# egor-achkasov/hermespy-rt

Hardware: AMD Instinct MI355X
Metric: resolved propagation paths/sec (higher is better)
Workload: dtype f32; 1 GPU; simple_street_canyon_with_cars.hrt, 1 TX + 4 RX, 4000000 rays/TX, 4 bounces, 3.5 GHz; parallelism=ray-sharded x1 (weak scaling), round-robin 4096-path granules, rays_total=4000000

## Files before the change

hermespy-rt_amd/csrc/hrt_kernels.hip:

```cpp
#include <hip/hip_runtime.h>
#include <string.h>

#include <stdint.h>
#include <stdio.h>
#include <stdlib.h>

#include "hrt_kparams.h"
#include "hrt_launch_dir.h"
#include "hrt_libm.h"

#pragma clang fp contract(off)

namespace {

constexpr float kEps = 1.1920928955078125e-07f;
constexpr float kOnePlusEps = 1.00000011920928955078125f;
constexpr float kPi = 3.14159265358979323846f;
constexpr float kC = 299792458.0f;
constexpr float kInvC = 1.0f / kC;
__device__ __forceinline__ float div_c(float a)
{
    const float q = a * kInvC;
    const float r = __builtin_fmaf(-q, kC, a);
    return __builtin_fmaf(r, kInvC, q);
// ... 434 lines not shown
                const float nt_s = xor_sign(nt, sg);                                            \
                rm |= HRT_BALLOT(nt_s < kK5 * a) | HRT_BALLOT(nt_s > (best * a) * kK2);         \
                if (rm != ~0ull) {                                                              \
                    HRT_STAT(kind, 5, 1);                                                       \
                    const float u = nu / det;                                                   \
                    const float v = nv / det;                                                   \
                    const float w = u + v;                                                      \
                    const float dist = nt / det;                                                \
                    const bool rej = (rm >> lane) & 1ull;                                       \
                    const bool miss = (det > -kEps && det < kEps) | (u < -kEps) |               \
                                      (u > kOnePlusEps) | (v < -kEps) | (w > kOnePlusEps);      \
                    const uint32_t oj = orig[(J)];         \
                    const bool take = !rej & !miss & (dist > kEps) &                            \
                                      ((dist < best) | ((dist == best) & (oj < who_o)));        \
                    best = take ? dist : best;                                                  \
                    who = take ? (J) : who;                                                     \
                    who_o = take ? oj : who_o;                                                  \
                }                                                                               \
            }                                                                                   \
        }                                                                                       \
    }

constexpr uint32_t kMaskRounds = 16;
constexpr uint32_t kCandBuf = 64u;
__host__ __device__ constexpr uint32_t wave_scratch4(bool cand_buf) { return 2u * kMaskRounds + (cand_buf ? 4u * kCandBuf : 0u); }

__device__ __forceinline__ uint32_t rxt_cell(F3 a)
{
    const float ax = fabsf(a.x), ay = fabsf(a.y), az = fabsf(a.z);
    uint32_t m = 0u;
    float major = a.x, c1 = a.y, c2 = a.z;
    if (ay > ax && ay >= az) { m = 1u; major = a.y; c1 = a.z; c2 = a.x; }
    else if (az > ax && az > ay) { m = 2u; major = a.z; c1 = a.x; c2 = a.y; }
    const float inv = __builtin_amdgcn_rcpf(major);
    const float u = c1 * inv, v = c2 * inv;
    int iu = (int)((u * 0.5f + 0.5f) * (float)HRT_RXT_N), iv = (int)((v * 0.5f + 0.5f) * (float)HRT_RXT_N);
    iu = iu < 0 ? 0 : (iu > HRT_RXT_N - 1 ? HRT_RXT_N - 1 : iu);
    iv = iv < 0 ? 0 : (iv > HRT_RXT_N - 1 ? HRT_RXT_N - 1 : iv);
    const uint32_t f = m + (major < 0.f ? 3u : 0u);
    return (f * HRT_RXT_N + (uint32_t)iv) * HRT_RXT_N + (uint32_t)iu;
}

__device__ __forceinline__ bool rxt_inside(const hrt_krxt &X, F3 o)
{
    const F3 dc = sub3(o, {X.cx, X.cy, X.cz});
    return fast_sqrt(fdot3(dc, dc)) * 1.0001f <= X.region_r;
}
__device__ __forceinline__ unsigned long long rxt_cell_load(const hrt_krxt &X, uint32_t apex_k, F3 d)
{
    return X.cell_mask[(uint64_t)apex_k * HRT_RXT_BINS + rxt_cell(d)];
}
template <typename TriPtr>
__device__ __forceinline__ Hit closest_hit_masked(TriPtr tri, const uint32_t *__restrict__ orig, const hrt_krxt &X,
                                                  uint32_t apex_k, uint32_t num_tri, F3 o, F3 d, bool valid,
                                                  uint32_t lane, [[maybe_unused]] int kind)
{
    float best = 1e9f;
    uint32_t who = HRT_NO_HIT, who_o = 0u;
    const unsigned long long inval = HRT_BALLOT(!valid);
    if (inval == ~0ull) return {who, best};
    unsigned long long mine = 0ull;
    if (valid) {
        mine = rxt_inside(X, o) ? rxt_cell_load(X, apex_k, d)
                                : (num_tri >= 64u ? ~0ull : ((1ull << num_tri) - 1ull));
    }
    unsigned long long m = wave_or64(mine);
    HRT_STAT(kind, 0, 1);
    HRT_STAT(kind, 1, 1);
    HRT_STAT(kind, 2, __popcll(m));
    while (m) {
        const uint32_t j = (uint32_t)__builtin_ctzll(m);
        m &= m - 1ull;
        HRT_STAGED_BODY(j)
    }
    return {who, best};
}

using Rsrc = __amdgpu_buffer_rsrc_t;
__device__ __forceinline__ Rsrc make_rsrc(const uint8_t *base)
{
    return __builtin_amdgcn_make_buffer_rsrc(const_cast<uint8_t *>(base), 0, 0xffffffff, 0x00020000);
}

__device__ __forceinline__ void wave_or256(uint32_t (&w)[8])
{
    uint32_t c[4];
#pragma unroll
    for (int k = 0; k < 4; ++k) {
        const auto r = __builtin_amdgcn_permlane32_swap(w[k], w[k + 4], false, false);
        c[k] = (uint32_t)r[0] | (uint32_t)r[1];
    }
    uint32_t e[2];
#pragma unroll
    for (int k = 0; k < 2; ++k) {
        const auto r = __builtin_amdgcn_permlane16_swap(c[k], c[k + 2], false, false);
        e[k] = (uint32_t)r[0] | (uint32_t)r[1];
    }
#define HRT_OR2(CTRL) "v_or_b32_dpp %0, %0, %0 " CTRL "\n" "v_or_b32_dpp %1, %1, %1 " CTRL "\n" "s_nop 0\n"
    asm volatile(
        "s_nop 4\n"
        HRT_OR2("row_shr:1 row_mask:0xf bank_mask:0xf")
        HRT_OR2("row_shr:2 row_mask:0xf bank_mask:0xf")
        HRT_OR2("row_shr:4 row_mask:0xf bank_mask:0xf")
        HRT_OR2("row_shr:8 row_mask:0xf bank_mask:0xf")
        "s_nop 1\n"
        : "+v"(e[0]), "+v"(e[1]));
#undef HRT_OR2
#pragma unroll
    for (int k = 0; k < 8; ++k) w[k] = (uint32_t)__builtin_amdgcn_readlane((int)e[k & 1], 15 + 16 * (k >> 1));
}

__device__ __forceinline__ F3 image_of(F3 t, float4 q0, float4 q2)
{
    const F3 n = {q2.y, q2.z, q2.w};
    const float dn = fdot3(sub3(t, {q0.x, q0.y, q0.z}), n);
    return {__builtin_fmaf(-2.f * dn, n.x, t.x), __builtin_fmaf(-2.f * dn, n.y, t.y), __builtin_fmaf(-2.f * dn, n.z, t.z)};
}

struct PatchRef { bool served; uint32_t off; };
__device__ __forceinline__ void patch_fetch(const hrt_kpatch &X, uint32_t num_tri, uint32_t htri, bool valid, float4 &p0, float4 &p1)
{
    p0 = make_float4(0.f, 0.f, 0.f, 0.f);
    p1 = p0;
    if (valid && htri < num_tri) {
        p0 = reinterpret_cast<const float4 *>(X.pdef)[2u * htri];
        p1 = reinterpret_cast<const float4 *>(X.pdef)[2u * htri + 1u];
    }
}
template <typename TriPtr>
__device__ __forceinline__ PatchRef patch_locate(TriPtr tri, const hrt_kpatch &X, uint32_t num_tri, uint32_t htri, F3 o,
                                                 const bool image, F3 apex, F3 d, const float4 p0, const float4 p1)
{
    PatchRef R = {false, 0u};
    if (htri < num_tri) {
        const float4 q0 = tri[HRT_ROW * htri], q2 = tri[HRT_ROW * htri + 2];
        const F3 sv = sub3(o, {q0.x, q0.y, q0.z});
        const float fu = fdot3(sv, {p0.x, p0.y, p0.z}), fv = fdot3(sv, {p1.x, p1.y, p1.z});
        const float hh = fdot3(sv, {q2.y, q2.z, q2.w});
        const uint32_t bits = __float_as_uint(p1.w), nu = bits & 0xffffu, nv = bits >> 16;
        R.served = (nu != 0u) & (fabsf(hh) <= X.hmax) & (fu >= -HRT_PATCH_ACCEPT) & (fv >= -HRT_PATCH_ACCEPT) &
                   (fu <= (float)nu + HRT_PATCH_ACCEPT) & (fv <= (float)nv + HRT_PATCH_ACCEPT);
        if (image) {
            const F3 im = image_of(apex, q0, q2);
            const F3 wv = sub3(o, im);
            const F3 cx = fcross3(wv, d);
            R.served &= (fdot3(cx, cx) <= 0.98f * X.ro_img * X.ro_img) && (fdot3(wv, d) > 0.f);
        }
        const uint32_t iu = min((uint32_t)max((int)floorf(fu), 0), nu - 1u);
        const uint32_t iv = min((uint32_t)max((int)floorf(fv), 0), nv - 1u);
        R.off = (__float_as_uint(p0.w) + iv * nu + iu) * (HRT_PATCH_WORDS * 8u);
    }
    return R;
}

__device__ __forceinline__ void patch_load(const hrt_kpatch &X, const PatchRef R, uint32_t apex_k, bool valid, uint32_t (&w)[8])
{
#pragma unroll
    for (int k = 0; k < 8; ++k) w[k] = 0u;
    if (valid && R.served) {
        const Rsrc mr = make_rsrc(reinterpret_cast<const uint8_t *>(X.mask));
        const uint32_t off = R.off + apex_k * X.num_patch * (HRT_PATCH_WORDS * 8u);
        const auto a = __builtin_amdgcn_raw_buffer_load_b128(mr, (int)off, 0, 0);
        const auto b = __builtin_amdgcn_raw_buffer_load_b128(mr, (int)(off + 16u), 0, 0);
        w[0] = (uint32_t)a[0]; w[1] = (uint32_t)a[1]; w[2] = (uint32_t)a[2]; w[3] = (uint32_t)a[3];
        w[4] = (uint32_t)b[0]; w[5] = (uint32_t)b[1]; w[6] = (uint32_t)b[2]; w[7] = (uint32_t)b[3];
    }
}
__device__ __forceinline__ bool patch_whole(const PatchRef R, bool valid) { return HRT_BALLOT(valid && !R.served) != 0ull; }

template <typename TriPtr, typename OrigPtr>
__device__ __forceinline__ Hit closest_hit_words(TriPtr tri, OrigPtr orig, uint32_t (&w)[8], const bool whole, uint32_t num_tri,
                                                 F3 o, F3 d, bool valid, uint32_t lane, [[maybe_unused]] int kind)
{
    float best = 1e9f;
    uint32_t who = HRT_NO_HIT, who_o = 0u;
    const unsigned long long inval = HRT_BALLOT(!valid);
    if (inval == ~0ull) return {who, best};
    wave_or256(w);
    if (whole) {
#pragma unroll
        for (int k = 0; k < 8; ++k)
            w[k] |= num_tri >= 32u * (uint32_t)(k + 1) ? ~0u : (num_tri > 32u * (uint32_t)k ? (1u << (num_tri - 32u * (uint32_t)k)) - 1u : 0u);
    }
    HRT_STAT(kind, 0, 1);
    HRT_STAT(kind, 1, 1);
#pragma unroll
    for (uint32_t r = 0; r < HRT_PATCH_WORDS; ++r) {
        unsigned long long m = ((unsigned long long)w[2u * r + 1u] << 32) | (unsigned long long)w[2u * r];
        HRT_STAT(kind, 2, __popcll(m));
        while (m) {
            const uint32_t j = r * 64u + (uint32_t)__builtin_ctzll(m);
            m &= m - 1ull;
            HRT_STAGED_BODY(j)
        }
    }
    return {who, best};
}

template <typename TriPtr, typename OrigPtr>
__device__ __forceinline__ Hit closest_hit_patch(TriPtr tri, OrigPtr orig, const hrt_kpatch &X,
                                                 const PatchRef R, uint32_t apex_k, uint32_t num_tri, F3 o, F3 d,
                                                 bool valid, uint32_t lane, [[maybe_unused]] int kind)
{
    uint32_t w[8];
    patch_load(X, R, apex_k, valid, w);
    HRT_STAT(kind, 6, (valid && R.served) ? 1 : 0);
    return closest_hit_words(tri, orig, w, patch_whole(R, valid), num_tri, o, d, valid, lane, kind);
}

__device__ __forceinline__ void txcell_load(const hrt_kpatch &X, uint32_t tx, F3 d, uint32_t (&w)[8])
{
    const Rsrc mr = make_rsrc(reinterpret_cast<const uint8_t *>(X.txcell));
    const uint32_t off = (tx * HRT_RXT_BINS + rxt_cell(d)) * (HRT_PATCH_WORDS * 8u);
    const auto a = __builtin_amdgcn_raw_buffer_load_b128(mr, (int)off, 0, 0);
    const auto b = __builtin_amdgcn_raw_buffer_load_b128(mr, (int)(off + 16u), 0, 0);
    w[0] = (uint32_t)a[0]; w[1] = (uint32_t)a[1]; w[2] = (uint32_t)a[2]; w[3] = (uint32_t)a[3];
    w[4] = (uint32_t)b[0]; w[5] = (uint32_t)b[1]; w[6] = (uint32_t)b[2]; w[7] = (uint32_t)b[3];
}

template <typename TriPtr, typename OrigPtr>
__device__ __forceinline__ Hit closest_hit_txcell(TriPtr tri, OrigPtr orig, const hrt_kpatch &X, uint32_t tx, uint32_t num_tri,
                                                  F3 o, F3 d, bool valid, uint32_t lane)
{
    uint32_t w[8];
#pragma unroll
    for (int k = 0; k < 8; ++k) w[k] = 0u;
    if (valid) txcell_load(X, tx, d, w);
    return closest_hit_words(tri, orig, w, false, num_tri, o, d, valid, lane, 0);
}

template <bool MULTI, typename TriPtr>
__device__ __forceinline__ Hit closest_hit_packet(TriPtr tri, const uint32_t *__restrict__ orig,
                                                  const hrt_krxt &X, uint32_t rxk,
                                                  uint32_t num_tri, F3 o, F3 d,
                                                  bool valid, uint32_t lane, const Ball &B,
                                                  const bool shadow, F3 apex,
                                                  unsigned long long *wmask, int kind)
{
    float best = 1e9f;
    uint32_t who = HRT_NO_HIT, who_o = 0u;
    const unsigned long long inval = HRT_BALLOT(!valid);
    if (inval == ~0ull) return {who, best};
    uint32_t n_items = num_tri;
    const uint16_t *list = nullptr;
    Packet P0 = packet_bounds(B, d, valid, shadow, apex);
    HRT_STAT(kind, 0, 1);
    HRT_STAT(kind, 1, P0.usable ? 1 : 0);
    if ((shadow || (kind == 0 && X.num_txt != 0u)) && X.enabled && P0.usable) {
        const F3 dc = sub3(B.c, {X.cx, X.cy, X.cz});
        const bool inside = fast_sqrt(fdot3(dc, dc)) * 1.0001f + B.r <= X.region_r;
        float ro_apex = P0.ro;
        if (!shadow) ro_apex += (fabsf(B.c.x - apex.x) + fabsf(B.c.y - apex.y)) + fabsf(B.c.z - apex.z);
        if (inside && P0.sina <= HRT_RXT_SIN_AQ && ro_apex <= X.ro_bin[rxk]) {
            const uint32_t cell = (uint32_t)__builtin_amdgcn_readfirstlane((int)rxt_cell(P0.ax));
            const uint32_t e0 = X.off[rxk * HRT_RXT_BINS + cell], e1 = X.off[rxk * HRT_RXT_BINS + cell + 1u];
            list = X.idx + e0;
            n_items = e1 - e0;
            HRT_STAT(kind, 6, 1);
            HRT_STAT(kind, 7, n_items);
        }
    }
// ... 1568 lines not shown
                stf(hit_out(P, b), H_OZ * cap4, k4, o.z);
                stf(hit_out(P, b), H_DX * cap4, k4, d.x);
                stf(hit_out(P, b), H_DY * cap4, k4, d.y);
                stf(hit_out(P, b), H_DZ * cap4, k4, d.z);
                stf(hit_out(P, b), H_A0 * cap4, k4, a0);
                stf(hit_out(P, b), H_A1 * cap4, k4, a1);
                stf(hit_out(P, b), H_A2 * cap4, k4, a2);
                stf(hit_out(P, b), H_A3 * cap4, k4, a3);
                stf(hit_out(P, b), H_TAU * cap4, k4, tau);
            }
        }
    }
}

__global__ __launch_bounds__(HRT_BLOCK, 8) void hrt_image_kernel(const hrt_kparams P, const uint32_t b)
{
    extern __shared__ float4 lds[];
    const uint32_t tid = threadIdx.x, lane = tid & 63u;
    const uint32_t *counts = reinterpret_cast<const uint32_t *>(P.ws + P.off_counts);
    if (counts[P.num_bounces + 1] & kErrVoid) return;
    const uint32_t n_in = counts[b];
    const uint32_t n_chunks = (n_in + HRT_BLOCK - 1) / HRT_BLOCK;
    if (blockIdx.x >= n_chunks) return;
    const uint32_t T = P.num_tri;
    const uint32_t cap4 = (uint32_t)P.cap * 4u;
    float4 *l_tri = lds;
    uint32_t *l_wcnt = reinterpret_cast<uint32_t *>(lds + HRT_ROW * T);
    const uint32_t pb = b - 1;
    F3 o, d;
    uint32_t htri, hray;
    float4 pd0, pd1;
    const auto load_state = [&](const uint32_t chunk) {
        const uint32_t i = chunk * HRT_BLOCK + tid;
        const uint32_t i4 = i * 4u;
        o = {0.f, 0.f, 0.f};
        d = {0.f, 0.f, 1.f};
        htri = 0u;
        hray = 0u;
        if (i < n_in) {
            htri = ldu(hit_blk(P, pb), H_TRI * cap4, i4);
            o = {ldf(hit_blk(P, pb), H_OX * cap4, i4), ldf(hit_blk(P, pb), H_OY * cap4, i4), ldf(hit_blk(P, pb), H_OZ * cap4, i4)};
            d = {ldf(hit_blk(P, pb), H_DX * cap4, i4), ldf(hit_blk(P, pb), H_DY * cap4, i4), ldf(hit_blk(P, pb), H_DZ * cap4, i4)};
            if (P.num_tx != 1u) hray = ldu(hit_blk(P, pb), H_RAY * cap4, i4);
        }
        patch_fetch(P.patch, T, htri, i < n_in, pd0, pd1);
    };
    {
        const float4 *g_tri = reinterpret_cast<const float4 *>(P.tri);
        float4 s_tri[kStageTri];
        copy16_request(s_tri, g_tri, HRT_ROW * T, tid);
        load_state(blockIdx.x);
        copy16_commit(s_tri, l_tri, g_tri, HRT_ROW * T, tid);
    }
    __syncthreads();
    const float4 *tri = l_tri;
    for (uint32_t chunk = blockIdx.x; chunk < n_chunks; chunk += gridDim.x) {
        const uint32_t i = chunk * HRT_BLOCK + tid;
        const uint32_t i4 = i * 4u;
        const bool valid = i < n_in;
        uint32_t tx = 0u;
        PatchRef ref = {false, 0u};
        if (valid) {
            if (P.num_tx != 1u) tx = min(hray / P.num_local, P.num_tx - 1u);
            ref = patch_locate(tri, P.patch, T, htri, o, true, {P.tx_pos[3 * tx], P.tx_pos[3 * tx + 1], P.tx_pos[3 * tx + 2]}, d, pd0, pd1);
        }
        const Hit h = closest_hit_patch(tri, P.acc.orig, P.patch, ref, P.num_rx + tx, T, o, d, valid, lane, 1);
        if (valid) {
            stu(res_blk(P, P.num_rx), 0u, i4, h.tri);
            stf(res_blk(P, P.num_rx), cap4, i4, h.t);
        }
        const unsigned long long hm = __ballot(valid && h.tri != HRT_NO_HIT);
        if (lane == 0) l_wcnt[tid >> 6] = (uint32_t)__popcll(hm);
        __syncthreads();
        if (tid == 0) {
            const uint32_t c = l_wcnt[0] + l_wcnt[1] + l_wcnt[2] + l_wcnt[3];
            reinterpret_cast<uint32_t *>(P.ws + P.off_chunk_cnt)[chunk] = c;
            atomicAdd(reinterpret_cast<uint32_t *>(P.ws + P.off_super_cnt) + (uint64_t)b * P.num_super + (chunk >> HRT_SUPER_SHIFT), c);
        }
        __syncthreads();
        if (chunk + gridDim.x < n_chunks) load_state(chunk + gridDim.x);
    }
}

#ifndef HRT_RECORDS_PREFETCH
#define HRT_RECORDS_PREFETCH 1
#endif
#ifndef HRT_RECORDS_WAVES
#define HRT_RECORDS_WAVES 6
#endif
__global__ __launch_bounds__(HRT_BLOCK, HRT_RECORDS_WAVES) void hrt_records_kernel(const hrt_kparams P, const uint32_t b)
{
    extern __shared__ float4 lds[];
    const uint32_t tid = threadIdx.x, lane = tid & 63u;
    const uint32_t *counts = reinterpret_cast<const uint32_t *>(P.ws + P.off_counts);
    if (counts[P.num_bounces + 1] & kErrVoid) return;
    const uint32_t n_in = counts[b];
    const uint32_t n_chunks = (n_in + HRT_BLOCK - 1) / HRT_BLOCK;
    if (blockIdx.x >= n_chunks) return;
    const uint32_t T = P.num_tri;
    const uint32_t cap4 = (uint32_t)P.cap * 4u;
    const Rsrc mesh_r = make_rsrc(reinterpret_cast<const uint8_t *>(P.mesh));
    float4 *l_tri = lds;
    float4 *l_rx = lds + HRT_ROW * T;
    float4 *l_mat = l_rx + P.num_rx;
    uint32_t *l_orig = reinterpret_cast<uint32_t *>(l_mat + 4u * HRT_NUM_MATERIALS);
    const uint32_t pb = b - 1;
    F3 o, d;
    uint32_t htri;
    float theta, tau, a0, a1, a2, a3;
    const auto load_state = [&](const uint32_t chunk) {
        const uint32_t i = chunk * HRT_BLOCK + tid;
        const uint32_t i4 = i * 4u;
        o = {0.f, 0.f, 0.f};
        d = {0.f, 0.f, 1.f};
        htri = 0u;
        theta = 0.f; tau = 0.f; a0 = 1.f; a1 = 0.f; a2 = 1.f; a3 = 0.f;
        if (i < n_in) {
            htri = ldu(hit_blk(P, pb), H_TRI * cap4, i4);
            theta = ldf(hit_blk(P, pb), H_THETA * cap4, i4);
            o = {ldf(hit_blk(P, pb), H_OX * cap4, i4), ldf(hit_blk(P, pb), H_OY * cap4, i4),
                 ldf(hit_blk(P, pb), H_OZ * cap4, i4)};
            d = {ldf(hit_blk(P, pb), H_DX * cap4, i4), ldf(hit_blk(P, pb), H_DY * cap4, i4),
                 ldf(hit_blk(P, pb), H_DZ * cap4, i4)};
            a0 = ldf(hit_blk(P, pb), H_A0 * cap4, i4);
            a1 = ldf(hit_blk(P, pb), H_A1 * cap4, i4);
            a2 = ldf(hit_blk(P, pb), H_A2 * cap4, i4);
            a3 = ldf(hit_blk(P, pb), H_A3 * cap4, i4);
            tau = ldf(hit_blk(P, pb), H_TAU * cap4, i4);
        }
    };
    {
        const float4 *g_tri = reinterpret_cast<const float4 *>(P.tri);
        const float4 *g_mat = reinterpret_cast<const float4 *>(P.mat);
        const auto ld_rx = [&](uint32_t k) { return stage_pos(P.rx_pos, k); };
        const auto ld_orig = [&](uint32_t k) { return P.acc.orig[k]; };
        float4 s_tri[kStageTri], s_rx[1], s_mat[1];
        uint32_t s_orig[1];
        copy16_request(s_tri, g_tri, HRT_ROW * T, tid);
        stage_load(s_rx, P.num_rx, tid, ld_rx);
        copy16_request(s_mat, g_mat, 4u * HRT_NUM_MATERIALS, tid);
        stage_load(s_orig, T, tid, ld_orig);
        load_state(blockIdx.x);
        copy16_commit(s_tri, l_tri, g_tri, HRT_ROW * T, tid);
        stage_store(l_rx, s_rx, P.num_rx, tid);
        copy16_commit(s_mat, l_mat, g_mat, 4u * HRT_NUM_MATERIALS, tid);
        stage_store(l_orig, s_orig, T, tid);
        stage_rest<1, 2>(l_rx, P.num_rx, tid, ld_rx);
        stage_rest<1, 2>(l_orig, T, tid, ld_orig);
    }
    __syncthreads();
    const float4 *tri = l_tri;
    for (uint32_t chunk = blockIdx.x; chunk < n_chunks; chunk += gridDim.x) {
        const uint32_t i = chunk * HRT_BLOCK + tid;
        const uint32_t i4 = i * 4u;
        const bool valid = i < n_in;
        F3 n = {0.f, 0.f, 1.f}, mvel = {0.f, 0.f, 0.f};
        float mat_s = 0.f, mat_alpha = 1.f;
        PatchRef ref = {false, 0u};
        if (valid) {
            float4 pd0, pd1;
            patch_fetch(P.patch, T, htri, true, pd0, pd1);
            float4 mm = make_float4(0.f, 0.f, 0.f, 0.f);
            if (htri < T) mm = gather4(mesh_r, HRT_MESH_FLOATS * 4u, __float_as_uint(tri[HRT_ROW * htri + 4].w), 0u);
            ref = patch_locate(tri, P.patch, T, htri, o, false, o, o, pd0, pd1);
            if (htri < T) {
                const float4 q2 = tri[HRT_ROW * htri + 2];
                n = {q2.y, q2.z, q2.w};
                mvel = {mm.x, mm.y, mm.z};
                const float4 m3 = l_mat[4u * __float_as_uint(mm.w) + 3u];
                mat_s = m3.x;
                mat_alpha = m3.y;
            }
        }
#if HRT_RECORDS_PREFETCH
        uint32_t wnext[8];
        patch_load(P.patch, ref, 0u, valid, wnext);
        const bool whole = patch_whole(ref, valid);
#endif
        for (uint32_t rx = 0; rx < P.num_rx; ++rx) {
            const float4 rp = l_rx[rx];
            float d2rx;
            F3 w = shadow_dir(o, {rp.x, rp.y, rp.z}, d2rx);
            if (!valid) w = {0.f, 0.f, 1.f};
#if HRT_RECORDS_PREFETCH
            uint32_t wcur[8];
#pragma unroll
            for (int q = 0; q < 8; ++q) wcur[q] = wnext[q];
            if (rx + 1u < P.num_rx) patch_load(P.patch, ref, rx + 1u, valid, wnext);
            const Hit h = closest_hit_words(tri, l_orig, wcur, whole, T, o, w, valid, lane, 2);
#else
            const Hit h = closest_hit_patch(tri, l_orig, P.patch, ref, rx, T, o, w, valid, lane, 2);
#endif
            bool unblocked = false;
            if (valid) {
                if (h.tri != HRT_NO_HIT) {
                    const float4 q2 = tri[HRT_ROW * h.tri + 2];
                    theta = incidence_angle({q2.y, q2.z, q2.w}, w);
                }
                if (h.tri != HRT_NO_HIT && h.t <= 1.f) {
                    stf(rec_blk(P, pb, rx), R_A0 * cap4, i4, 0.f);
                    stf(rec_blk(P, pb, rx), R_A1 * cap4, i4, 0.f);
                    stf(rec_blk(P, pb, rx), R_A2 * cap4, i4, 0.f);
                    stf(rec_blk(P, pb, rx), R_A3 * cap4, i4, 0.f);
                    stf(rec_blk(P, pb, rx), R_TAU * cap4, i4, 0.f);
                } else {
                    unblocked = true;
                    const float th_s = acos_f_ool(dot3(w, n));
                    const float4 S = scatter_pattern(mat_s, mat_alpha, th_s, theta);
                    float o0 = a0 * S.x - a1 * S.y;
                    float o1 = a0 * S.y + a1 * S.x;
                    float o2 = a2 * S.z - a3 * S.w;
                    float o3 = a2 * S.w + a3 * S.z;
                    float f2 = P.fsl_mult * d2rx;
                    f2 *= f2;
                    if (f2 > 1.f) { o0 /= f2; o1 /= f2; o2 /= f2; o3 /= f2; }
                    stf(rec_blk(P, pb, rx), R_A0 * cap4, i4, o0);
                    stf(rec_blk(P, pb, rx), R_A1 * cap4, i4, o1);
                    stf(rec_blk(P, pb, rx), R_A2 * cap4, i4, o2);
                    stf(rec_blk(P, pb, rx), R_A3 * cap4, i4, o3);
                    stf(rec_blk(P, pb, rx), R_TAU * cap4, i4, tau + div_c(d2rx));
                    stf(rec_blk(P, pb, rx), R_DX * cap4, i4, -w.x);
                    stf(rec_blk(P, pb, rx), R_DY * cap4, i4, -w.y);
                    stf(rec_blk(P, pb, rx), R_DZ * cap4, i4, -w.z);
                    stf(rec_blk(P, pb, rx), R_DFS * cap4, i4, dot3(sub3(w, d), mvel) * P.dop_mult);
                }
            }
            const unsigned long long m = __ballot(unblocked);
            if (lane == 0 && valid) mask_words(P, pb, rx)[i >> 6] = m;
        }
        if (chunk + gridDim.x < n_chunks) load_state(chunk + gridDim.x);
    }
}

__device__ __forceinline__ void los_pairs(const hrt_kparams &P, const uint32_t block);

constexpr uint32_t kLbDone = 1u << 31;

__device__ __forceinline__ uint32_t lb_load(const uint32_t *p)
{
    return __hip_atomic_load(p, __ATOMIC_RELAXED, __HIP_MEMORY_SCOPE_AGENT);
}
__device__ __forceinline__ void lb_store(uint32_t *p, uint32_t v)
{
    __hip_atomic_store(p, v, __ATOMIC_RELAXED, __HIP_MEMORY_SCOPE_AGENT);
}

struct LbWords { uint32_t *chunk, *group, *super; };
__device__ __forceinline__ LbWords lb_words(const hrt_kparams &P, uint32_t b)
{
    LbWords W;
    W.chunk = reinterpret_cast<uint32_t *>(P.ws + P.off_lb) + (uint64_t)b * P.lb_stride;
    W.group = W.chunk + P.lb_chunks;
    W.super = W.group + P.lb_chunks / 64u;
    return W;
}

constexpr uint32_t kLbAbort = 0xffffffffu;
__device__ __forceinline__ void give_up(uint32_t *err_word, uint32_t *host_flag, uint32_t err_bit)
{
    atomicOr(err_word, err_bit);
    if (host_flag)
        __hip_atomic_store(host_flag + (err_bit == kErrChainTimeout ? 1 : 0), 1u, __ATOMIC_RELAXED, __HIP_MEMORY_SCOPE_SYSTEM);
}
__device__ __forceinline__ uint32_t lb_exclusive(const LbWords &W, uint32_t chunk, uint32_t c, uint32_t lane,
                                                 uint32_t *err_word, uint32_t *host_flag, const uint32_t max_polls,
                                                 const uint32_t err_bit = kErrFuseTimeout)
{
    uint32_t polls = 0u;
    const uint32_t g = chunk >> 6, sg = chunk >> 12;
    const bool want_c = (g << 6) + lane < chunk, want_g = (sg << 6) + lane < g;
    const bool want_s0 = lane < sg, want_s1 = lane + 64u < sg;
    bool g_owed = (chunk & 63u) == 63u, s_owed = (chunk & 4095u) == 4095u;
    for (;;) {
        const uint32_t cw = want_c ? lb_load(W.chunk + (g << 6) + lane) : kLbDone;
        const uint32_t gw = want_g ? lb_load(W.group + (sg << 6) + lane) : kLbDone;
        const uint32_t s0 = want_s0 ? lb_load(W.super + lane) : kLbDone;
        const uint32_t s1 = want_s1 ? lb_load(W.super + lane + 64u) : kLbDone;
        const bool ok_c = HRT_BALLOT(!(cw & kLbDone)) == 0ull, ok_g = HRT_BALLOT(!(gw & kLbDone)) == 0ull;
        const bool ok_s = HRT_BALLOT(!(s0 & s1 & kLbDone)) == 0ull;
        uint32_t sum_c = 0u, sum_g = 0u;
        if (ok_c && (g_owed || (ok_g && (s_owed || ok_s)))) sum_c = wave_sum_u32(cw & ~kLbDone);
        if (ok_c && g_owed) {
            if (lane == 0) lb_store(W.group + g, kLbDone | (sum_c + c));
            g_owed = false;
        }
        if (ok_c && ok_g && (s_owed || ok_s)) sum_g = wave_sum_u32(gw & ~kLbDone);
        if (ok_c && ok_g && s_owed) {
            if (lane == 0) lb_store(W.super + sg, kLbDone | (sum_g + sum_c + c));
            s_owed = false;
        }
        if (ok_c && ok_g && ok_s) return sum_c + sum_g + wave_sum_u32((s0 & ~kLbDone) + (s1 & ~kLbDone));
        if (lb_load(err_word) & kErrVoid) return kLbAbort;
        if (++polls > max_polls) {
            if (lane == 0) give_up(err_word, host_flag, err_bit);
            return kLbAbort;
        }
        __builtin_amdgcn_s_sleep(4);
    }
}

constexpr uint32_t kLdsTx = 64u;
struct FusedLds {
    float4 *tri, *leaf, *rx, *wleaf, *mat, *tx;
    float2 *tg;
    unsigned long long *mask;
    uint32_t *wcnt;
};
template <bool TRI_IN_LDS, bool CAND_BUF>
__device__ __forceinline__ FusedLds fused_lds(float4 *lds, uint32_t T, uint32_t n_leaf, uint32_t num_rx, uint32_t wave)
{
    FusedLds L;
// ... 1057 lines not shown
    const uint64_t T = P->num_tri;
    const uint64_t tri_bytes = T * HRT_TRI_FLOATS * 4u + ((T + 1u) / 2u) * 16u +
                               (uint64_t)P->acc.num_leaf * HRT_NODE_FLOATS * 4u;
    const bool in_lds = T * HRT_TRI_FLOATS * 4u <= lds_max && tri_bytes <= 144u * 1024u;
    const bool one_block = P->num_tri <= kMaskRounds * 64u;
    const bool trees = P->acc.big && (variant >= 4) && variant != 9;
    const bool flat = variant == 2 || variant == 3 || (variant == 7 && !trees && one_block);
    return bounce != 0 && P->patch.mask != nullptr && in_lds && flat && one_block && !walks_fine(P);
}

int hrt_hip_launch_trace(const hrt_kparams *P_in, uint32_t bounce, void *stream)
{
    hrt_kparams Pc = *P_in;
    Pc.cnt_per_wave = walks_fine(P_in) ? 1u : 0u;
    const hrt_kparams *P = &Pc;
    const uint64_t n_max = (bounce == 0) ? P->n0 : P->cap;
    const uint64_t kinds = (bounce == 0) ? 1u : (bounce < P->num_bounces ? P->num_rx + 1u : P->num_rx);
    uint64_t blocks = ((n_max + HRT_BLOCK - 1) / HRT_BLOCK) * kinds;
    const uint64_t max_grid = P->tune.trace_grid ? P->tune.trace_grid : HRT_TRACE_GRID;
    if (blocks > max_grid) blocks = max_grid;
    if (blocks == 0) blocks = 1;
    const int variant = P->tune.variant;
    const uint64_t T = P->num_tri;
    const uint64_t tri_bytes = T * HRT_TRI_FLOATS * 4u + ((T + 1u) / 2u) * 16u +
                               (uint64_t)P->acc.num_leaf * HRT_NODE_FLOATS * 4u;
    const uint64_t lds_max = P->tune.lds_tri_bytes_max;
    const bool in_lds = T * HRT_TRI_FLOATS * 4u <= lds_max && tri_bytes <= 144u * 1024u;
    const bool one_block = P->num_tri <= kMaskRounds * 64u;
    const bool fine_pre = !in_lds && !(P->acc.big && variant >= 4 && variant != 9) && P->acc.fine != nullptr &&
                          (variant == 7 || variant == 9);
    const size_t lds = (in_lds ? (size_t)tri_bytes : 0u) + (size_t)P->num_rx * 16u +
                       (HRT_BLOCK / 64u) * (kMaskRounds * 8u + wave_scratch4(fine_pre) * 16u) + 16u;
    hipStream_t st = (hipStream_t)stream;
    hipError_t err = hipSuccess;
    const uint32_t nb = (uint32_t)blocks;
    const bool trees = P->acc.big && (variant >= 4) && variant != 9;
    const bool flat = variant == 2 || variant == 3 || (variant == 7 && !trees && one_block);
    const bool fine = !in_lds && !trees && P->acc.fine != nullptr && (variant == 7 || variant == 9);
    if (fine) {
        launch_trace_t<false, 9>(P, bounce, nb, lds, st, &err);
        if (err == hipSuccess && P->wide_cap != 0u) {
            const uint64_t wide_grid = P->tune.wide_grid ? P->tune.wide_grid : kWideGrid;
            hipLaunchKernelGGL(hrt_wide_kernel, dim3((uint32_t)wide_grid), dim3(HRT_BLOCK), 0, st, *P, bounce);
            hipLaunchKernelGGL(hrt_wide_finish_kernel, dim3(256), dim3(HRT_BLOCK), 0, st, *P, bounce);
        }
    } else if (in_lds) {
        if (variant == 0) launch_trace_t<true, 0>(P, bounce, nb, lds, st, &err);
        else if (variant == 1) launch_trace_t<true, 1>(P, bounce, nb, lds, st, &err);
        else if (flat) {
            if (records_in_own_kernel(P, bounce)) {
                if (bounce < P->num_bounces) {
                    uint64_t pblocks = (n_max + HRT_BLOCK - 1) / HRT_BLOCK;
                    if (pblocks > max_grid) pblocks = max_grid;
                    if (bounce == 1 && P->patch.num_img != 0u)
                        hipLaunchKernelGGL(hrt_image_kernel, dim3((uint32_t)pblocks), dim3(HRT_BLOCK),
                                           (size_t)T * HRT_TRI_FLOATS * 4u + 16u, st, *P, bounce);
                    else
                        launch_trace_t<true, 2>(P, bounce, (uint32_t)pblocks, lds, st, &err);
                }
            } else if (one_block) launch_trace_t<true, 2>(P, bounce, nb, lds, st, &err);
            else launch_trace_t<true, 3>(P, bounce, nb, lds, st, &err);
        } else if (trees) launch_trace_t<true, 6>(P, bounce, nb, lds, st, &err);
        else if (one_block) launch_trace_t<true, 4>(P, bounce, nb, lds, st, &err);
        else launch_trace_t<true, 5>(P, bounce, nb, lds, st, &err);
    } else {
        if (variant == 0) launch_trace_t<false, 0>(P, bounce, nb, lds, st, &err);
        else if (variant == 1) launch_trace_t<false, 1>(P, bounce, nb, lds, st, &err);
        else if (flat) launch_trace_t<false, 3>(P, bounce, nb, lds, st, &err);
        else if (trees) launch_trace_t<false, 6>(P, bounce, nb, lds, st, &err);
        else launch_trace_t<false, 5>(P, bounce, nb, lds, st, &err);
    }
    if (err != hipSuccess) return (int)err;
    return (int)hipGetLastError();
}

int hrt_hip_launch_records(const hrt_kparams *P, uint32_t bounce, void *stream)
{
    if (!records_in_own_kernel(P, bounce)) return -1;
    const uint64_t max_grid = P->tune.trace_grid ? P->tune.trace_grid : HRT_TRACE_GRID;
    const uint64_t T = P->num_tri;
    uint64_t rblocks = (P->cap + HRT_BLOCK - 1) / HRT_BLOCK;
    if (rblocks > 2u * max_grid) rblocks = 2u * max_grid;
    const size_t rlds = (size_t)T * HRT_TRI_FLOATS * 4u + (size_t)P->num_rx * 16u +
                        (size_t)(HRT_NUM_MATERIALS * HRT_MAT_FLOATS * 4u) + (size_t)T * 4u;
    if (rlds > 64u * 1024u) return (int)hipErrorInvalidValue;
    hipLaunchKernelGGL(hrt_records_kernel, dim3((uint32_t)rblocks), dim3(HRT_BLOCK), rlds, (hipStream_t)stream, *P, bounce);
    return (int)hipGetLastError();
}

int hrt_hip_launch_shade(const hrt_kparams *P_in, uint32_t bounce, void *stream)
{
    hrt_kparams Pc = *P_in;
    Pc.cnt_per_wave = walks_fine(P_in) ? 1u : 0u;
    Pc.records_done = records_in_own_kernel(P_in, bounce) ? 1u : 0u;
    if (Pc.records_done && bounce >= Pc.num_bounces) return 0;
    const hrt_kparams *P = &Pc;
    const uint64_t n_max = (bounce == 0) ? P->n0 : P->cap;
    uint64_t blocks = (n_max + HRT_BLOCK - 1) / HRT_BLOCK;
    const uint64_t max_grid = P->tune.shade_grid ? P->tune.shade_grid : HRT_SHADE_GRID;
    if (blocks > max_grid) blocks = max_grid;
    if (blocks == 0) blocks = 1;
    const size_t lds0 = (size_t)(HRT_NUM_MATERIALS * HRT_MAT_FLOATS * 4u) + (size_t)P->num_rx * 16u + 32u;
    const uint64_t nlds_off = P->tune.shade_global_normals;
    if (!nlds_off && P->num_tri <= kShadeLdsTri && P->num_mesh <= kShadeLdsMesh)
        hipLaunchKernelGGL(hrt_shade_kernel<true>, dim3((uint32_t)blocks), dim3(HRT_BLOCK),
                           lds0 + ((size_t)P->num_tri + P->num_mesh) * 16u, (hipStream_t)stream, *P, bounce);
    else
        hipLaunchKernelGGL(hrt_shade_kernel<false>, dim3((uint32_t)blocks), dim3(HRT_BLOCK), lds0,
                           (hipStream_t)stream, *P, bounce);
    return (int)hipGetLastError();
}

int hrt_hip_launch_fused(const hrt_kparams *P_in, uint32_t bounce, void *stream)
{
    hrt_kparams Pc = *P_in;
#ifdef HRT_PHASE_STATS
    Pc.phase_bounce = (uint32_t)env_u64("HRT_PHASE_BOUNCE", 0);
#endif
    Pc.records_done = records_in_own_kernel(P_in, bounce) ? 1u : 0u;
    if (bounce != 0) Pc.los_blocks = 0;
    else if (Pc.los_blocks) Pc.los_blocks = (Pc.num_rx * Pc.num_tx + HRT_BLOCK / 64u - 1u) / (HRT_BLOCK / 64u);
    const hrt_kparams *P = &Pc;
    if (P->cap / HRT_BLOCK + 1u > P->lb_chunks) return (int)hipErrorInvalidValue;
    const int variant = P->tune.variant;
    const uint64_t T = P->num_tri;
    const uint64_t tri_bytes = T * HRT_TRI_FLOATS * 4u + ((T + 1u) / 2u) * 16u +
                               (uint64_t)P->acc.num_leaf * HRT_NODE_FLOATS * 4u;
    const uint64_t lds_max = P->tune.lds_tri_bytes_max;
    const bool in_lds = T * HRT_TRI_FLOATS * 4u <= lds_max && tri_bytes <= 144u * 1024u;
    const bool one_block = P->num_tri <= kMaskRounds * 64u;
    const bool fine_pre = !in_lds && !(P->acc.big && variant >= 4 && variant != 9) && P->acc.fine != nullptr &&
                          (variant == 7 || variant == 9);
    const size_t lds = (in_lds ? (size_t)tri_bytes : 0u) + (size_t)P->num_rx * 16u +
                       (HRT_BLOCK / 64u) * (kMaskRounds * 8u + wave_scratch4(fine_pre) * 16u) + 64u * 4u +
                       (size_t)(HRT_NUM_MATERIALS * HRT_MAT_FLOATS * 4u) + kLdsTx * 16u;
    hipStream_t st = (hipStream_t)stream;
    hipError_t err = hipSuccess;
    const uint64_t staged_max = P->tune.fuse_staged_max_tri;
    const bool trees = P->acc.big && (variant >= 4) && variant != 9;
    const bool flat = variant == 2 || variant == 3 || (variant == 7 && !trees && one_block);
    const bool staged = variant == 1 || (variant == 7 && T <= staged_max);
    const bool fine = !in_lds && !trees && P->acc.fine != nullptr && (variant == 7 || variant == 9);
    if (fine) return -1;
    else if (in_lds) {
        if (variant == 0) launch_fused_t<true, 0>(P, bounce, lds, st, &err);
        else if (staged) launch_fused_t<true, 1>(P, bounce, lds, st, &err);
        else if (flat) {
            if (one_block) launch_fused_t<true, 2>(P, bounce, lds, st, &err);
            else launch_fused_t<true, 3>(P, bounce, lds, st, &err);
        } else if (trees) launch_fused_t<true, 6>(P, bounce, lds, st, &err);
        else if (one_block) launch_fused_t<true, 4>(P, bounce, lds, st, &err);
        else launch_fused_t<true, 5>(P, bounce, lds, st, &err);
    } else {
        if (variant == 0) launch_fused_t<false, 0>(P, bounce, lds, st, &err);
        else if (staged) launch_fused_t<false, 1>(P, bounce, lds, st, &err);
        else if (flat) launch_fused_t<false, 3>(P, bounce, lds, st, &err);
        else if (trees) launch_fused_t<false, 6>(P, bounce, lds, st, &err);
        else launch_fused_t<false, 5>(P, bounce, lds, st, &err);
    }
    if (err == hipErrorNotSupported) return -1;
    if (err != hipSuccess) return (int)err;
    return (int)hipGetLastError();
}

int hrt_hip_launch_chain(const hrt_kparams *P_in, uint32_t b0, void *stream)
{
    if (b0 == 0 || b0 > P_in->num_bounces) return -1;
// ... 260 lines not shown
```

Measured before the change: 27.10 billion paths/s.

## Batch per-RX patch mask loads and wave-OR reductions into LDS slots in records kernel

In the records kernel, per-receiver candidate-mask loads are now issued in flights of several receivers at once. Each mask is reduced across the wave with the permlane/DPP OR, and the row results are stored into a per-wave LDS slot. The per-receiver shadow test then reads the precomputed union mask from LDS through readfirstlane, skipping the in-loop wave_or256. This replaces the single-step prefetch and aims to raise memory-level parallelism and take the reduction latency off the critical per-receiver path. The cost is extra LDS per block, more registers held for masks in flight, and wave-level fences.

```diff
diff --git a/hermespy-rt_amd/csrc/hrt_kernels.hip b/hermespy-rt_amd/csrc/hrt_kernels.hip
--- a/hermespy-rt_amd/csrc/hrt_kernels.hip
+++ b/hermespy-rt_amd/csrc/hrt_kernels.hip
@@ -540,7 +540,7 @@
     return __builtin_amdgcn_make_buffer_rsrc(const_cast<uint8_t *>(base), 0, 0xffffffff, 0x00020000);
 }
 
-__device__ __forceinline__ void wave_or256(uint32_t (&w)[8])
+__device__ __forceinline__ void wave_or256_rows(const uint32_t (&w)[8], uint32_t (&e)[2])
 {
     uint32_t c[4];
 #pragma unroll
@@ -548,7 +548,6 @@
         const auto r = __builtin_amdgcn_permlane32_swap(w[k], w[k + 4], false, false);
         c[k] = (uint32_t)r[0] | (uint32_t)r[1];
     }
-    uint32_t e[2];
 #pragma unroll
     for (int k = 0; k < 2; ++k) {
         const auto r = __builtin_amdgcn_permlane16_swap(c[k], c[k + 2], false, false);
@@ -564,6 +563,11 @@
         "s_nop 1\n"
         : "+v"(e[0]), "+v"(e[1]));
 #undef HRT_OR2
+}
+__device__ __forceinline__ void wave_or256(uint32_t (&w)[8])
+{
+    uint32_t e[2];
+    wave_or256_rows(w, e);
 #pragma unroll
     for (int k = 0; k < 8; ++k) w[k] = (uint32_t)__builtin_amdgcn_readlane((int)e[k & 1], 15 + 16 * (k >> 1));
 }
@@ -626,7 +630,7 @@
 }
 __device__ __forceinline__ bool patch_whole(const PatchRef R, bool valid) { return HRT_BALLOT(valid && !R.served) != 0ull; }
 
-template <typename TriPtr, typename OrigPtr>
+template <bool UNION = true, typename TriPtr, typename OrigPtr>
 __device__ __forceinline__ Hit closest_hit_words(TriPtr tri, OrigPtr orig, uint32_t (&w)[8], const bool whole, uint32_t num_tri,
                                                  F3 o, F3 d, bool valid, uint32_t lane, [[maybe_unused]] int kind)
 {
@@ -634,7 +638,7 @@
     uint32_t who = HRT_NO_HIT, who_o = 0u;
     const unsigned long long inval = HRT_BALLOT(!valid);
     if (inval == ~0ull) return {who, best};
-    wave_or256(w);
+    if (UNION) wave_or256(w);
     if (whole) {
 #pragma unroll
         for (int k = 0; k < 8; ++k)
@@ -2369,12 +2373,15 @@
     }
 }
 
-#ifndef HRT_RECORDS_PREFETCH
-#define HRT_RECORDS_PREFETCH 1
-#endif
 #ifndef HRT_RECORDS_WAVES
 #define HRT_RECORDS_WAVES 6
 #endif
+#ifndef HRT_RECORDS_FLIGHT
+#define HRT_RECORDS_FLIGHT 4
+#endif
+constexpr uint32_t kRecBatch = 8u, kRecFlight = HRT_RECORDS_FLIGHT;
+static_assert(kRecBatch % kRecFlight == 0u, "a flight must not write past the batch's slots");
+constexpr uint32_t kRecSlotBytes = (HRT_BLOCK / 64u) * kRecBatch * 32u;
 __global__ __launch_bounds__(HRT_BLOCK, HRT_RECORDS_WAVES) void hrt_records_kernel(const hrt_kparams P, const uint32_t b)
 {
     extern __shared__ float4 lds[];
@@ -2391,6 +2398,7 @@
     float4 *l_rx = lds + HRT_ROW * T;
     float4 *l_mat = l_rx + P.num_rx;
     uint32_t *l_orig = reinterpret_cast<uint32_t *>(l_mat + 4u * HRT_NUM_MATERIALS);
+    uint32_t *l_slot = l_orig + ((T + 3u) & ~3u) + (tid >> 6) * (kRecBatch * 8u);
     const uint32_t pb = b - 1;
     F3 o, d;
     uint32_t htri;
@@ -2459,61 +2467,78 @@
                 mat_alpha = m3.y;
             }
         }
-#if HRT_RECORDS_PREFETCH
-        uint32_t wnext[8];
-        patch_load(P.patch, ref, 0u, valid, wnext);
         const bool whole = patch_whole(ref, valid);
-#endif
-        for (uint32_t rx = 0; rx < P.num_rx; ++rx) {
-            const float4 rp = l_rx[rx];
-            float d2rx;
-            F3 w = shadow_dir(o, {rp.x, rp.y, rp.z}, d2rx);
-            if (!valid) w = {0.f, 0.f, 1.f};
-#if HRT_RECORDS_PREFETCH
-            uint32_t wcur[8];
+        const bool any = HRT_BALLOT(valid) != 0ull;
+        for (uint32_t rx0 = 0; rx0 < P.num_rx; rx0 += kRecBatch) {
+            const uint32_t nrx = min(P.num_rx - rx0, kRecBatch);
+            if (any) {
+                for (uint32_t k = 0; k < nrx; k += kRecFlight) {
+                    uint32_t wm[kRecFlight][8];
 #pragma unroll
-            for (int q = 0; q < 8; ++q) wcur[q] = wnext[q];
-            if (rx + 1u < P.num_rx) patch_load(P.patch, ref, rx + 1u, valid, wnext);
-            const Hit h = closest_hit_words(tri, l_orig, wcur, whole, T, o, w, valid, lane, 2);
-#else
-            const Hit h = closest_hit_patch(tri, l_orig, P.patch, ref, rx, T, o, w, valid, lane, 2);
-#endif
-            bool unblocked = false;
-            if (valid) {
-                if (h.tri != HRT_NO_HIT) {
-                    const float4 q2 = tri[HRT_ROW * h.tri + 2];
-                    theta = incidence_angle({q2.y, q2.z, q2.w}, w);
+                    for (uint32_t f = 0; f < kRecFlight; ++f)
+                        patch_load(P.patch, ref, rx0 + k + f, valid && k + f < nrx, wm[f]);
+#pragma unroll
+                    for (uint32_t f = 0; f < kRecFlight; ++f) {
+                        uint32_t e[2];
+                        wave_or256_rows(wm[f], e);
+                        if ((lane & 15u) == 15u)
+                            reinterpret_cast<uint2 *>(l_slot + 8u * (k + f))[lane >> 4] = make_uint2(e[0], e[1]);
+                    }
                 }
-                if (h.tri != HRT_NO_HIT && h.t <= 1.f) {
-                    stf(rec_blk(P, pb, rx), R_A0 * cap4, i4, 0.f);
-                    stf(rec_blk(P, pb, rx), R_A1 * cap4, i4, 0.f);
-                    stf(rec_blk(P, pb, rx), R_A2 * cap4, i4, 0.f);
-                    stf(rec_blk(P, pb, rx), R_A3 * cap4, i4, 0.f);
-                    stf(rec_blk(P, pb, rx), R_TAU * cap4, i4, 0.f);
-                } else {
-                    unblocked = true;
-                    const float th_s = acos_f_ool(dot3(w, n));
-                    const float4 S = scatter_pattern(mat_s, mat_alpha, th_s, theta);
-                    float o0 = a0 * S.x - a1 * S.y;
-                    float o1 = a0 * S.y + a1 * S.x;
-                    float o2 = a2 * S.z - a3 * S.w;
-                    float o3 = a2 * S.w + a3 * S.z;
-                    float f2 = P.fsl_mult * d2rx;
-                    f2 *= f2;
-                    if (f2 > 1.f) { o0 /= f2; o1 /= f2; o2 /= f2; o3 /= f2; }
-                    stf(rec_blk(P, pb, rx), R_A0 * cap4, i4, o0);
-                    stf(rec_blk(P, pb, rx), R_A1 * cap4, i4, o1);
-                    stf(rec_blk(P, pb, rx), R_A2 * cap4, i4, o2);
-                    stf(rec_blk(P, pb, rx), R_A3 * cap4, i4, o3);
-                    stf(rec_blk(P, pb, rx), R_TAU * cap4, i4, tau + div_c(d2rx));
-                    stf(rec_blk(P, pb, rx), R_DX * cap4, i4, -w.x);
-                    stf(rec_blk(P, pb, rx), R_DY * cap4, i4, -w.y);
-                    stf(rec_blk(P, pb, rx), R_DZ * cap4, i4, -w.z);
-                    stf(rec_blk(P, pb, rx), R_DFS * cap4, i4, dot3(sub3(w, d), mvel) * P.dop_mult);
+            }
+            __builtin_amdgcn_fence(__ATOMIC_ACQ_REL, "wavefront");
+            __builtin_amdgcn_wave_barrier();
+            for (uint32_t rx = rx0; rx < rx0 + nrx; ++rx) {
+                const float4 rp = l_rx[rx];
+                float d2rx;
+                F3 w = shadow_dir(o, {rp.x, rp.y, rp.z}, d2rx);
+                if (!valid) w = {0.f, 0.f, 1.f};
+                uint32_t wu[8];
+                {
+                    const uint4 ua = reinterpret_cast<const uint4 *>(l_slot + 8u * (rx - rx0))[0];
+                    const uint4 ub = reinterpret_cast<const uint4 *>(l_slot + 8u * (rx - rx0))[1];
+                    const uint32_t uv[8] = {ua.x, ua.y, ua.z, ua.w, ub.x, ub.y, ub.z, ub.w};
+#pragma unroll
+                    for (int q = 0; q < 8; ++q) wu[q] = (uint32_t)__builtin_amdgcn_readfirstlane((int)uv[q]);
                 }
-            }
-            const unsigned long long m = __ballot(unblocked);
-            if (lane == 0 && valid) mask_words(P, pb, rx)[i >> 6] = m;
+                const Hit h = closest_hit_words<false>(tri, l_orig, wu, whole, T, o, w, valid, lane, 2);
+                bool unblocked = false;
+                if (valid) {
+                    if (h.tri != HRT_NO_HIT) {
+                        const float4 q2 = tri[HRT_ROW * h.tri + 2];
+                        theta = incidence_angle({q2.y, q2.z, q2.w}, w);
+                    }
+                    if (h.tri != HRT_NO_HIT && h.t <= 1.f) {
+                        stf(rec_blk(P, pb, rx), R_A0 * cap4, i4, 0.f);
+                        stf(rec_blk(P, pb, rx), R_A1 * cap4, i4, 0.f);
+                        stf(rec_blk(P, pb, rx), R_A2 * cap4, i4, 0.f);
+                        stf(rec_blk(P, pb, rx), R_A3 * cap4, i4, 0.f);
+                        stf(rec_blk(P, pb, rx), R_TAU * cap4, i4, 0.f);
+                    } else {
+                        unblocked = true;
+                        const float th_s = acos_f_ool(dot3(w, n));
+                        const float4 S = scatter_pattern(mat_s, mat_alpha, th_s, theta);
+                        float o0 = a0 * S.x - a1 * S.y;
+                        float o1 = a0 * S.y + a1 * S.x;
+                        float o2 = a2 * S.z - a3 * S.w;
+                        float o3 = a2 * S.w + a3 * S.z;
+                        float f2 = P.fsl_mult * d2rx;
+                        f2 *= f2;
+                        if (f2 > 1.f) { o0 /= f2; o1 /= f2; o2 /= f2; o3 /= f2; }
+                        stf(rec_blk(P, pb, rx), R_A0 * cap4, i4, o0);
+                        stf(rec_blk(P, pb, rx), R_A1 * cap4, i4, o1);
+                        stf(rec_blk(P, pb, rx), R_A2 * cap4, i4, o2);
+                        stf(rec_blk(P, pb, rx), R_A3 * cap4, i4, o3);
+                        stf(rec_blk(P, pb, rx), R_TAU * cap4, i4, tau + div_c(d2rx));
+                        stf(rec_blk(P, pb, rx), R_DX * cap4, i4, -w.x);
+                        stf(rec_blk(P, pb, rx), R_DY * cap4, i4, -w.y);
+                        stf(rec_blk(P, pb, rx), R_DZ * cap4, i4, -w.z);
+                        stf(rec_blk(P, pb, rx), R_DFS * cap4, i4, dot3(sub3(w, d), mvel) * P.dop_mult);
+                    }
+                }
+                const unsigned long long m = __ballot(unblocked);
+                if (lane == 0 && valid) mask_words(P, pb, rx)[i >> 6] = m;
+            }
         }
         if (chunk + gridDim.x < n_chunks) load_state(chunk + gridDim.x);
     }
@@ -3737,7 +3762,8 @@
     uint64_t rblocks = (P->cap + HRT_BLOCK - 1) / HRT_BLOCK;
     if (rblocks > 2u * max_grid) rblocks = 2u * max_grid;
     const size_t rlds = (size_t)T * HRT_TRI_FLOATS * 4u + (size_t)P->num_rx * 16u +
-                        (size_t)(HRT_NUM_MATERIALS * HRT_MAT_FLOATS * 4u) + (size_t)T * 4u;
+                        (size_t)(HRT_NUM_MATERIALS * HRT_MAT_FLOATS * 4u) + (((size_t)T * 4u + 15u) & ~(size_t)15u) +
+                        (size_t)kRecSlotBytes;
     if (rlds > 64u * 1024u) return (int)hipErrorInvalidValue;
     hipLaunchKernelGGL(hrt_records_kernel, dim3((uint32_t)rblocks), dim3(HRT_BLOCK), rlds, (hipStream_t)stream, *P, bounce);
     return (int)hipGetLastError();
```

Result: no change. 27.18 billion paths/s, median of 6 (+0.3%).
